# mlpc-ucsd/BDM

Measured on AMD Instinct MI355X. Metric: sampled shapes/sec (4096 pts, 1000 DDPM steps), higher is better.
Workload: dtype f32

## Files before the change

bdm_amd/csrc/common.h:

```cpp
#pragma once
#include <stdlib.h>
#include <hip/hip_runtime.h>
#include <stdint.h>

#define BDM_OK 0
#define BDM_ERR_ARG 1
#define BDM_ERR_LAUNCH 2
#define BDM_ERR_UNSUPPORTED 3

namespace bdm {

void set_error(const char *fmt, ...);

inline int launch_status(const char *what) {
  hipError_t e = hipGetLastError();
  if (e != hipSuccess) {
    set_error("%s: %s (HIP's per-thread last-error state: raised by this launch or left by an earlier unchecked call)",
              what, hipGetErrorString(e));
    return BDM_ERR_LAUNCH;
  }
  return BDM_OK;
}

#define BDM_REQUIRE(cond, ...)      \
// ... 116 lines not shown
__device__ __forceinline__ double wave_sum_bfly(double v) {
  BDM_FULL_WAVE();
  v = row16_sum(v);
  return (readlane_f64(v, 0) + readlane_f64(v, 16)) + (readlane_f64(v, 32) + readlane_f64(v, 48));
}
__device__ __forceinline__ float wave_max(float v) {
  BDM_FULL_WAVE();
  v = fmaxf(v, dpp_f32(v, BDM_DPP_QUAD_XOR1));
  v = fmaxf(v, dpp_f32(v, BDM_DPP_QUAD_XOR2));
  v = fmaxf(v, dpp_f32(v, BDM_DPP_ROW_HALF_MIRROR));
  v = fmaxf(v, dpp_f32(v, BDM_DPP_ROW_MIRROR));
  return fmaxf(fmaxf(readlane_f32(v, 0), readlane_f32(v, 16)), fmaxf(readlane_f32(v, 32), readlane_f32(v, 48)));
}
#endif

struct VoxWs {
  int *start;
  int *tmp;
  int *sorted;
};
static inline VoxWs vox_ws(void *ws, int b, int n, int r3) {
  VoxWs w;
  w.start = (int *)ws;
  w.tmp = w.start + (size_t)b * r3;
  w.sorted = w.tmp + (size_t)b * n;
  return w;
}

#if defined(__HIPCC__)
__device__ __forceinline__ float swishf(float x) {
  return x * __builtin_amdgcn_rcpf(1.0f + __builtin_amdgcn_exp2f(-x * 1.44269504088896340736f));
}
#endif

#if defined(__HIPCC__)
__device__ __forceinline__ void lds_settle(float &a, float &b) { asm volatile("s_waitcnt lgkmcnt(0)" : "+v"(a), "+v"(b)); }
__device__ __forceinline__ void lds_settle8(float (&v)[8]) {
  asm volatile("s_waitcnt lgkmcnt(0)" : "+v"(v[0]), "+v"(v[1]), "+v"(v[2]), "+v"(v[3]), "+v"(v[4]), "+v"(v[5]), "+v"(v[6]), "+v"(v[7]));
}
// ... 4 lines not shown
```

bdm_amd/csrc/pvcnn_ops.hip:

```cpp
#include <stdarg.h>
#include <stdio.h>

#include <stdlib.h>

#include "../../include/bdm_hip.h"
#include "common.h"

#pragma clang fp contract(off)

namespace bdm {
static thread_local char g_err[512] = "";
void set_error(const char *fmt, ...) {
  va_list ap;
  va_start(ap, fmt);
  vsnprintf(g_err, sizeof(g_err), fmt, ap);
  va_end(ap);
}
}

extern "C" const char *bdm_last_error(void) { return bdm::g_err; }
extern "C" int bdm_abi_version(void) { return 4; }

using namespace bdm;

// ... 497 lines not shown
    if (ci < c_a) {
      const float *fr = fa + (size_t)bi * bs_a + (size_t)ci * ld_a;
      out0[(size_t)bi * bs_0 + (size_t)ci * ld_0 + j] =
          __fadd_rn(__fadd_rn(__fmul_rn(fr[i0], w0), __fmul_rn(fr[i1], w1)), __fmul_rn(fr[i2], w2));
    } else if (ci < c_a + c_s) {
      out0[(size_t)bi * bs_0 + (size_t)ci * ld_0 + j] = fs[(size_t)bi * bs_s + (size_t)(ci - c_a) * ld_s + j];
    } else {
      const int ct = ci - c_a - c_s;
      const float *fr = ft + (size_t)bi * bs_t + (size_t)ct * ld_t;
      out1[(size_t)bi * bs_1 + (size_t)ct * ld_1 + j] =
          __fadd_rn(__fadd_rn(__fmul_rn(fr[i0], w0), __fmul_rn(fr[i1], w1)), __fmul_rn(fr[i2], w2));
    }
  }
}

extern "C" int bdm_fp_assemble(int b, int m, int n, const int *indices, const float *weights, int c_a, const float *fa,
                               long long bs_a, int ld_a, int c_s, const float *fs, long long bs_s, int ld_s, int c_t,
                               const float *ft, long long bs_t, int ld_t, float *out0, long long bs_0, int ld_0, float *out1,
                               long long bs_1, int ld_1, void *stream) {
  BDM_REQUIRE(b >= 0 && m >= 1 && n >= 0 && c_a >= 0 && c_s >= 0 && c_t >= 0, "fp_assemble: bad sizes");
  if (b == 0 || n == 0 || c_a + c_s + c_t == 0) return BDM_OK;
  const int c = c_a + c_s + c_t;
  dim3 grid(cdiv(n, 256), c < 64 ? c : 64, b);
  hipLaunchKernelGGL(fp_assemble_kernel, grid, dim3(256), 0, (hipStream_t)stream, n, c_a, fa, bs_a, ld_a, c_s, fs, bs_s, ld_s, c_t,
                     ft, bs_t, ld_t, indices, weights, out0, bs_0, ld_0, out1, bs_1, ld_1);
  return launch_status("fp_assemble");
}

extern "C" int bdm_three_nn_interpolate_forward(int b, int c, int m, int n, const float *points,
                                                const float *centers, const float *features, float *out,
                                                int *indices, float *weights, void *stream) {
  int rc = bdm_three_nn_search(b, m, n, points, centers, indices, weights, stream);
  if (rc) return rc;
  return bdm_three_nn_apply(b, c, m, n, features, (long long)c * m, m, indices, weights, out,
                            (long long)c * n, n, stream);
}

extern "C" size_t bdm_voxelize_workspace_bytes(int b, int n, int r) {
  return sizeof(int) * ((size_t)b * r * r * r + 2 * (size_t)b * n);
}

__global__ void vox_plan_kernel(int n, int r, const int *__restrict__ coords, int *__restrict__ ind,
                                int *__restrict__ cnt, int *__restrict__ start, int *__restrict__ tmp,
                                int *__restrict__ sorted, int n_max, int *__restrict__ occ_index,
                                int *__restrict__ occ_list, int *__restrict__ n_occ, unsigned char *__restrict__ rowocc) {
  extern __shared__ int lcnt[];
  __shared__ int wave_tot[16];
  const int r2 = r * r, r3 = r2 * r;
  const int bi = blockIdx.x, tid = threadIdx.x, T = blockDim.x, lane = tid & 63, wave = tid >> 6;
  const int *vx = coords + (size_t)bi * 3 * n, *vy = vx + n, *vz = vy + n;
  int *id = ind + (size_t)bi * n;
  int *gc = cnt + (size_t)bi * r3;
  int *gs = start + (size_t)bi * r3;
  int *tp = tmp + (size_t)bi * n;
  int *so = sorted + (size_t)bi * n;

  for (int v = tid; v < r3; v += T) lcnt[v] = 0;
  __syncthreads();
  for (int i = tid; i < n; i += T) {
    const int v = vx[i] * r2 + vy[i] * r + vz[i];
// ... 15 lines not shown
  __syncthreads();
  int wave_off = 0;
  for (int w = 0; w < wave; ++w) wave_off += wave_tot[w];
  int run = wave_off + incl - local;
  for (int v = lo; v < hi; ++v) { const int cv = lcnt[v]; gs[v] = run; lcnt[v] = run; run += cv; }
  __syncthreads();
  for (int i = tid; i < n; i += T) tp[atomicAdd(&lcnt[id[i]], 1)] = i;
  __syncthreads();
  for (int i = tid; i < n; i += T) {
    const int v = id[i];
    const int s = gs[v], cv = gc[v];
    int rank = 0;
    for (int q = 0; q < cv; ++q) rank += tp[s + q] < i;
    so[s + rank] = i;
  }
  if (occ_index == nullptr) return;
  __syncthreads();
  int *oi = occ_index + (size_t)bi * r3;
  int *ol = occ_list + (size_t)bi * n_max;
  int occ_local = 0;
  for (int v = lo; v < hi; ++v) occ_local += gc[v] > 0;
  int oincl = occ_local;
#pragma unroll
  for (int o = 1; o < 64; o <<= 1) {
    const int t = __shfl_up(oincl, o, 64);
    if (lane >= o) oincl += t;
  }
  __syncthreads();
  if (lane == 63) wave_tot[wave] = oincl;
  __syncthreads();
  int off = 0, total = 0;
  for (int w = 0; w < (T >> 6); ++w) { if (w < wave) off += wave_tot[w]; total += wave_tot[w]; }
  int orun = off + oincl - occ_local;
  for (int v = lo; v < hi; ++v) {
    if (gc[v] > 0) { oi[v] = orun; ol[orun] = v; ++orun; }
    else oi[v] = -1;
  }
  if (tid == 0) n_occ[bi] = total;
  for (int row = tid; row < r2; row += T) {
    int any = 0;
    for (int z = 0; z < r; ++z) any |= gc[row * r + z];
    rowocc[(size_t)bi * r2 + row] = any ? 1 : 0;
  }
}

template <int CS>
__global__ __launch_bounds__(1024) void vox_plan_slab_kernel(int n, int r, int slabs, const int *__restrict__ coords,
                                                             int *__restrict__ ind, int *__restrict__ cnt,
                                                             int *__restrict__ start, int *__restrict__ sorted, int n_max,
                                                             int *__restrict__ occ_index, int *__restrict__ occ_list,
                                                             int *__restrict__ n_occ, unsigned char *__restrict__ rowocc) {
  extern __shared__ int slab_smem[];
  constexpr int T = 1024, PER = CS / T;
  static_assert(CS % T == 0 && PER >= 1, "slab size must be a multiple of the workgroup size");
  const int r2 = r * r, r3 = r2 * r;
  int *lcnt = slab_smem;
  unsigned *bits = reinterpret_cast<unsigned *>(lcnt + CS);
  int *lbeg = reinterpret_cast<int *>(bits + r3 / 32);
  int *lst = lbeg + CS;
  __shared__ int red[16], red2[16];
  const int bi = blockIdx.x / slabs, sl = blockIdx.x % slabs, tid = threadIdx.x, lane = tid & 63, wave = tid >> 6;
  const int lo_cell = sl * CS;
  const int *vx = coords + (size_t)bi * 3 * n, *vy = vx + n, *vz = vy + n;
  int *id = ind + (size_t)bi * n;
  int *gc = cnt + (size_t)bi * r3, *gs = start + (size_t)bi * r3, *so = sorted + (size_t)bi * n;

  for (int v = tid; v < CS; v += T) lcnt[v] = 0;
  for (int w = tid; w < r3 / 32; w += T) bits[w] = 0u;
  __syncthreads();
  int before = 0;
  for (int i = tid; i < n; i += T) {
    const int v = vx[i] * r2 + vy[i] * r + vz[i];
    if (sl == 0) id[i] = v;
    atomicOr(&bits[v >> 5], 1u << (v & 31));
// ... 6 lines not shown
  __syncthreads();
  int occ_before = 0, occ_total = 0;
  for (int w = tid; w < r3 / 32; w += T) {
    const int pc = __popc(bits[w]);
    occ_total += pc;
    occ_before += (w < lo_cell / 32) ? pc : 0;
  }
#pragma unroll
  for (int o = 32; o > 0; o >>= 1) { occ_before += __shfl_xor(occ_before, o, 64); occ_total += __shfl_xor(occ_total, o, 64); }
  __shared__ int red3[16];
  if (lane == 0) { red2[wave] = occ_before; red3[wave] = occ_total; }
  __syncthreads();
  int point_base = 0, occ_base = 0, occ_all = 0;
  for (int w = 0; w < T / 64; ++w) { point_base += red[w]; occ_base += red2[w]; occ_all += red3[w]; }
  if (sl == 0 && tid == 0 && n_occ != nullptr) n_occ[bi] = occ_all;
  __syncthreads();

  int cv[PER], local = 0, olocal = 0;
#pragma unroll
  for (int j = 0; j < PER; ++j) { cv[j] = lcnt[tid * PER + j]; local += cv[j]; olocal += cv[j] > 0; }
  int incl = local, oincl = olocal;
#pragma unroll
  for (int o = 1; o < 64; o <<= 1) {
    const int t1 = __shfl_up(incl, o, 64), t2 = __shfl_up(oincl, o, 64);
    if (lane >= o) { incl += t1; oincl += t2; }
  }
  if (lane == 63) { red[wave] = incl; red2[wave] = oincl; }
  __syncthreads();
  int woff = 0, owoff = 0;
  for (int w = 0; w < wave; ++w) { woff += red[w]; owoff += red2[w]; }
  int run = woff + incl - local;
  int orun = occ_base + owoff + oincl - olocal;
#pragma unroll
  for (int j = 0; j < PER; ++j) {
    const int v = lo_cell + tid * PER + j;
    gc[v] = cv[j];
    gs[v] = point_base + run;
    lcnt[tid * PER + j] = run;
    lbeg[tid * PER + j] = run;
    if (occ_index != nullptr) {
      if (cv[j] > 0) { occ_index[(size_t)bi * r3 + v] = orun; occ_list[(size_t)bi * n_max + orun] = v; ++orun; }
      else occ_index[(size_t)bi * r3 + v] = -1;
    }
    run += cv[j];
  }
  if (rowocc != nullptr) {
    const int any = local > 0;
    const unsigned long long m = __ballot(any);
    constexpr int TPR_MAX = 64;
    const int tpr = r / PER;
    if (tpr <= TPR_MAX && (lane % tpr) == 0) {
      const unsigned long long rowmask = ((tpr == 64 ? ~0ull : ((1ull << tpr) - 1ull)) << lane);
      const int row = (lo_cell + tid * PER) / r;
      rowocc[(size_t)bi * r2 + row] = (m & rowmask) ? 1 : 0;
    }
  }
  __syncthreads();
  for (int i = tid; i < n; i += T) {
    const int v = vx[i] * r2 + vy[i] * r + vz[i];
    if (v >= lo_cell && v < lo_cell + CS) lst[atomicAdd(&lcnt[v - lo_cell], 1)] = i;
  }
  __syncthreads();
  for (int i = tid; i < n; i += T) {
    const int v = vx[i] * r2 + vy[i] * r + vz[i];
    if (v >= lo_cell && v < lo_cell + CS) {
      const int s0 = lbeg[v - lo_cell], cvv = lcnt[v - lo_cell] - s0;
      int rank = 0;
      for (int q = 0; q < cvv; ++q) rank += lst[s0 + q] < i;
      so[point_base + s0 + rank] = i;
    }
  }
}

__global__ void vox_reduce_kernel(int c, int n, int r3, const float *__restrict__ feat,
                                  const int *__restrict__ cnt, const int *__restrict__ start,
                                  const int *__restrict__ sorted, float *__restrict__ out) {
  const int v = blockIdx.x * blockDim.x + threadIdx.x;
  const int bi = blockIdx.z;
  if (v >= r3) return;
  const int cv = cnt[(size_t)bi * r3 + v];
  const int s = start[(size_t)bi * r3 + v];
  const int *so = sorted + (size_t)bi * n + s;
  const float inv = cv > 0 ? (float)(1.0 / (double)(float)cv) : 0.f;
  for (int ci = blockIdx.y; ci < c; ci += gridDim.y) {
// ... 4 lines not shown
  }
}

static bool vox_plan_slabs() { return bdm_staging_choice() != 0; }

extern "C" int bdm_voxelize_plan(int b, int n, int r, const int *coords, int *ind, int *cnt, void *workspace,
                                 void *stream) {
  BDM_REQUIRE(b >= 0 && n >= 1 && r >= 1 && r <= 32, "voxelize_plan: bad sizes (r<=32 supported)");
  BDM_REQUIRE(workspace != nullptr, "voxelize_plan: workspace is NULL");
  if (b == 0) return BDM_OK;
  const int r3 = r * r * r;
  VoxWs w = vox_ws(workspace, b, n, r3);
  const size_t smem = (size_t)r3 * sizeof(int);
  BDM_ALLOW_LDS(vox_plan_kernel, smem);
  hipLaunchKernelGGL(vox_plan_kernel, dim3(b), dim3(1024), smem, (hipStream_t)stream, n, r, coords, ind, cnt, w.start,
                     w.tmp, w.sorted, 0, (int *)nullptr, (int *)nullptr, (int *)nullptr, (unsigned char *)nullptr);
  return launch_status("vox_plan");
}

extern "C" int bdm_voxelize_plan_full(int b, int n, int r, int n_max, const int *coords, int *ind, int *cnt, void *workspace,
                                      int *occ_index, int *occ_list, int *n_occ, unsigned char *rowocc, void *stream) {
  BDM_REQUIRE(b >= 0 && n >= 1 && r >= 1 && r <= 32 && n_max >= 1, "voxelize_plan_full: bad sizes (r<=32 supported)");
  BDM_REQUIRE(workspace && occ_index && occ_list && n_occ && rowocc, "voxelize_plan_full: NULL buffer");
  if (b == 0) return BDM_OK;
  const int r3 = r * r * r;
  VoxWs w = vox_ws(workspace, b, n, r3);
  if (r == 32 && n <= 24576 && vox_plan_slabs()) {
    const size_t sm = sizeof(int) * (2 * 4096 + (size_t)r3 / 32 + (size_t)n);
    BDM_ALLOW_LDS(vox_plan_slab_kernel<4096>, sm);
    hipLaunchKernelGGL(vox_plan_slab_kernel<4096>, dim3(b * 8), dim3(1024), sm, (hipStream_t)stream, n, r, 8, coords, ind, cnt,
                       w.start, w.sorted, n_max, occ_index, occ_list, n_occ, rowocc);
    return launch_status("vox_plan_full");
  }
  const size_t smem = (size_t)r3 * sizeof(int);
  BDM_ALLOW_LDS(vox_plan_kernel, smem);
  hipLaunchKernelGGL(vox_plan_kernel, dim3(b), dim3(1024), smem, (hipStream_t)stream, n, r, coords, ind, cnt, w.start,
                     w.tmp, w.sorted, n_max, occ_index, occ_list, n_occ, rowocc);
  return launch_status("vox_plan_full");
}

extern "C" int bdm_avg_voxelize_forward(int b, int c, int n, int r, const float *features, const int *coords,
                                        float *out, int *ind, int *cnt, void *workspace, void *stream) {
  BDM_REQUIRE(b >= 0 && c >= 0 && n >= 1 && r >= 1 && r <= 32, "avg_voxelize: bad sizes (r<=32 supported)");
  if (b == 0) return BDM_OK;
  hipStream_t s = (hipStream_t)stream;
  const int r3 = r * r * r;
  int rc = bdm_voxelize_plan(b, n, r, coords, ind, cnt, workspace, stream);
  VoxWs w = vox_ws(workspace, b, n, r3);
  if (rc || c == 0) return rc;
  dim3 grid(cdiv(r3, 256), c < 64 ? c : 64, b);
  hipLaunchKernelGGL(vox_reduce_kernel, grid, dim3(256), 0, s, c, n, r3, features, cnt, w.start, w.sorted, out);
  return launch_status("vox_reduce");
// ... 44 lines not shown
```

bdm_amd/csrc/sparse_conv.hip:

```cpp
#include <stdlib.h>

#include "../../include/bdm_hip.h"
#include "common.h"
#include "s3_split.h"

using namespace bdm;

__global__ void vox_compact_kernel(int r3, int n_max, const int *__restrict__ cnt, int *__restrict__ occ_index,
                                   int *__restrict__ occ_list, int *__restrict__ n_occ) {
  __shared__ int wave_tot[16];
  const int bi = blockIdx.x, tid = threadIdx.x, T = blockDim.x, lane = tid & 63, wave = tid >> 6;
  const int *c = cnt + (size_t)bi * r3;
  int *oi = occ_index + (size_t)bi * r3;
  int *ol = occ_list + (size_t)bi * n_max;
  const int per = (r3 + T - 1) / T;
  const int lo = min(tid * per, r3), hi = min(lo + per, r3);
  int local = 0;
  for (int v = lo; v < hi; ++v) local += c[v] > 0;
  int incl = local;
#pragma unroll
  for (int o = 1; o < 64; o <<= 1) {
    const int t = __shfl_up(incl, o, 64);
    if (lane >= o) incl += t;
  }
// ... 128 lines not shown
#pragma unroll
        for (int j = 0; j < 8; ++j)
          if (j < nch) acc[j] = acc[j] + v[u][j] * inv;
      }
  }
  store_s3(xs + ((size_t)bi * G + g) * 3 * (size_t)n_max * 8, (size_t)k, (size_t)n_max, acc);
}

template <int OUT>
__global__ __launch_bounds__(1024) void sparse_vox_features_lds_kernel(int c, int n, int r3, int n_max, int G, int ksplit,
                                                                       int cells_per,
                                                                       const float *__restrict__ feat, long long bs_f, int ld_f,
                                                                       const int *__restrict__ cnt, const int *__restrict__ start,
                                                                       const int *__restrict__ sorted,
                                                                       const int *__restrict__ occ_list,
                                                                       const int *__restrict__ n_occ, void *__restrict__ outp,
                                                                       unsigned *__restrict__ amax) {
#pragma clang fp contract(off)
  extern __shared__ float frows[];
  constexpr int CPT = 4;
  const int unit = blockIdx.x / ksplit, k0 = (blockIdx.x % ksplit) * cells_per, bi = unit / G, g = unit % G;
  const int tid = threadIdx.x, T = blockDim.x;
  const int nocc = min(n_occ[bi], n_max);
  const int lim = min(OUT == 0 ? min((nocc + 127) & ~127, n_max) : n_max, k0 + cells_per);
  if (k0 >= lim) return;
  const int nch = min(8, c - g * 8);
  const float *fb = feat + (size_t)bi * bs_f + (size_t)g * 8 * ld_f;
  const bool vec = (n & 3) == 0 && (ld_f & 3) == 0 && ((reinterpret_cast<size_t>(fb) & 15) == 0) && (n >> 2) <= T;
  const int n4 = n >> 2;
  float4 rowv[8];
  if (vec) {
#pragma unroll
    for (int j = 0; j < 8; ++j)
      rowv[j] = reinterpret_cast<const float4 *>(fb + (size_t)min(j, nch - 1) * ld_f)[min(tid, n4 - 1)];
  }
  int cs[CPT], cc[CPT];
#pragma unroll
  for (int i = 0; i < CPT; ++i) {
    const int k = k0 + tid + i * T;
    cs[i] = 0; cc[i] = 0;
    if (k < nocc && k < lim) {
      const int v = occ_list[(size_t)bi * n_max + k];
      cc[i] = cnt[(size_t)bi * r3 + v];
      cs[i] = start[(size_t)bi * r3 + v];
    }
  }
  int pre[CPT][4];
#pragma unroll
  for (int i = 0; i < CPT; ++i) {
    const int *so = sorted + (size_t)bi * n + cs[i];
#pragma unroll
    for (int u = 0; u < 4; ++u) pre[i][u] = cc[i] > 0 ? so[min(u, cc[i] - 1)] : 0;
  }
  if (vec) {
    if (tid < n4) {
#pragma unroll
      for (int j = 0; j < 8; ++j)
        reinterpret_cast<float4 *>(frows + j * n)[tid] = j < nch ? rowv[j] : make_float4(0.f, 0.f, 0.f, 0.f);
    }
  } else if ((n & 3) == 0 && (ld_f & 3) == 0 && ((reinterpret_cast<size_t>(fb) & 15) == 0)) {
#pragma unroll
    for (int j = 0; j < 8; ++j) {
      const float4 *src = reinterpret_cast<const float4 *>(fb + (size_t)min(j, nch - 1) * ld_f);
      float4 *dst = reinterpret_cast<float4 *>(frows + j * n);
      for (int p = tid; p < n4; p += T) {
        const float4 v = src[p];
        dst[p] = j < nch ? v : make_float4(0.f, 0.f, 0.f, 0.f);
// ... 6 lines not shown
  __syncthreads();
  float m = 0.f;
#pragma unroll
  for (int i = 0; i < CPT; ++i) {
    const int k = k0 + tid + i * T;
    if (k >= lim) continue;
    const int cv = cc[i];
    const int *so = sorted + (size_t)bi * n + cs[i];
    const float inv = cv > 0 ? (float)(1.0 / (double)(float)cv) : 0.f;
    float acc[8];
#pragma unroll
    for (int j = 0; j < 8; ++j) acc[j] = 0.f;
    for (int q0 = 0; q0 < cv; q0 += 4) {
      int p[4];
#pragma unroll
      for (int u = 0; u < 4; ++u) p[u] = q0 == 0 ? pre[i][u] : so[min(q0 + u, cv - 1)];
#pragma unroll
      for (int u = 0; u < 4; ++u)
        if (q0 + u < cv) {
#pragma unroll
          for (int j = 0; j < 8; ++j) acc[j] = acc[j] + frows[j * n + p[u]] * inv;
        }
    }
    if (OUT == 0) {
      store_s3(reinterpret_cast<unsigned short *>(outp) + ((size_t)bi * G + g) * 3 * (size_t)n_max * 8, (size_t)k, (size_t)n_max, acc);
    } else {
      float4 *o = reinterpret_cast<float4 *>(outp) + (((size_t)bi * G + g) * n_max + k) * 2;
      o[0] = make_float4(acc[0], acc[1], acc[2], acc[3]);
      o[1] = make_float4(acc[4], acc[5], acc[6], acc[7]);
#pragma unroll
      for (int j = 0; j < 8; ++j) m = fmaxf(m, fabsf(acc[j]));
    }
  }
  if (OUT == 1) {
    m = wave_max(m);
    if ((tid & 63) == 0 && m > 0.f) atomicMax(amax + bi, __float_as_uint(m));
  }
}

bool bdm_sparse_features_lds_launch(int out_kind, int b, int c, int n, int r3, int n_max, const float *features, long long bs_f,
                                    int ld_f, const int *cnt, const int *start, const int *sorted, const int *occ_list,
                                    const int *n_occ, void *out, unsigned *amax, hipStream_t stream, int *rc) {
  if (bdm_staging_choice() == 0 || n > 4096 || n_max > 4096) return false;
  const int G = (c + 7) / 8, units = b * G;
  const int ksplit = 1;
  const int cells_per = ((n_max + ksplit - 1) / ksplit + 63) & ~63;
  const int T = cells_per > 1024 ? 1024 : 256;
  const size_t smem = sizeof(float) * 8 * (size_t)n;
  *rc = BDM_OK;
  if (out_kind == 0) {
    static int granted0[16] = {0};
    int dev = 0;
    (void)hipGetDevice(&dev);
    if (smem > 48 * 1024 && (dev < 0 || dev >= 16 || granted0[dev] < (int)smem)) {
      hipError_t e = hipFuncSetAttribute((const void *)sparse_vox_features_lds_kernel<0>, hipFuncAttributeMaxDynamicSharedMemorySize, (int)smem);
      if (e != hipSuccess) return false;
      if (dev >= 0 && dev < 16) granted0[dev] = (int)smem;
    }
    hipLaunchKernelGGL(sparse_vox_features_lds_kernel<0>, dim3(units * ksplit), dim3(T), smem, stream, c, n, r3, n_max, G, ksplit,
                       cells_per, features, bs_f, ld_f, cnt, start, sorted, occ_list, n_occ, out, amax);
  } else {
    static int granted1[16] = {0};
    int dev = 0;
    (void)hipGetDevice(&dev);
    if (smem > 48 * 1024 && (dev < 0 || dev >= 16 || granted1[dev] < (int)smem)) {
      hipError_t e = hipFuncSetAttribute((const void *)sparse_vox_features_lds_kernel<1>, hipFuncAttributeMaxDynamicSharedMemorySize, (int)smem);
      if (e != hipSuccess) return false;
      if (dev >= 0 && dev < 16) granted1[dev] = (int)smem;
    }
    hipLaunchKernelGGL(sparse_vox_features_lds_kernel<1>, dim3(units * ksplit), dim3(T), smem, stream, c, n, r3, n_max, G, ksplit,
                       cells_per, features, bs_f, ld_f, cnt, start, sorted, occ_list, n_occ, out, amax);
  }
  return true;
}

extern "C" int bdm_sparse_voxel_features_s3(int b, int c, int n, int r, int n_max, const float *features, long long bs_f,
                                            int ld_f, const int *cnt, const void *plan_workspace, const int *occ_list,
                                            const int *n_occ, void *xs, void *stream) {
  BDM_REQUIRE(b >= 0 && c >= 1 && n >= 1 && r >= 1 && n_max >= 1, "sparse_voxel_features_s3: bad sizes");
  if (b == 0) return BDM_OK;
  const int r3 = r * r * r;
  VoxWs w = vox_ws(const_cast<void *>(plan_workspace), b, n, r3);
  int rc_lds = BDM_OK;
  if (bdm_sparse_features_lds_launch(0, b, c, n, r3, n_max, features, bs_f, ld_f, cnt, w.start, w.sorted, occ_list, n_occ, xs, nullptr,
                                     (hipStream_t)stream, &rc_lds))
    return launch_status("sparse_voxel_features_s3");
  const int G = (c + 7) / 8, units = b * G, kblocks = cdiv(n_max, 128);
  hipLaunchKernelGGL(sparse_vox_features_s3_kernel, dim3(cdiv(units, 8) * 8 * kblocks), dim3(128), 0, (hipStream_t)stream, c,
                     n, r3, n_max, G, units, kblocks, features, bs_f, ld_f, cnt, w.start, w.sorted, occ_list, n_occ,
                     (unsigned short *)xs);
  return launch_status("sparse_voxel_features_s3");
}

__global__ void sparse_pack_s3_kernel(int cout, int cin, const float *__restrict__ w, unsigned short *__restrict__ ws) {
  const int n27 = 27 * cout, G = (cin + 7) / 8;
  const long long total = (long long)G * n27;
  for (long long e = (long long)blockIdx.x * blockDim.x + threadIdx.x; e < total; e += (long long)gridDim.x * blockDim.x) {
    const int g = (int)(e / n27), col = (int)(e % n27), tap = col / cout, co = col % cout;
    float v[8];
// ... 429 lines not shown
```

bdm_amd/csrc/sparse_conv_h2.hip:

```cpp
#include <stdlib.h>

#include "../../include/bdm_hip.h"
#include "common.h"

using namespace bdm;

#include "sparse_h2_common.h"

bool bdm_sparse_features_lds_launch(int out_kind, int b, int c, int n, int r3, int n_max, const float *features, long long bs_f,
                                    int ld_f, const int *cnt, const int *start, const int *sorted, const int *occ_list,
                                    const int *n_occ, void *out, unsigned *amax, hipStream_t stream, int *rc);

__global__ void sparse_vox_features_f32_kernel(int c, int n, int r3, int n_max, int G, int units, int kblocks,
                                               const float *__restrict__ feat, long long bs_f, int ld_f,
                                               const int *__restrict__ cnt, const int *__restrict__ start,
                                               const int *__restrict__ sorted, const int *__restrict__ occ_list,
                                               const int *__restrict__ n_occ, float4 *__restrict__ xr,
                                               unsigned *__restrict__ amax) {
#pragma clang fp contract(off)
  const int wg = blockIdx.x, span = 8 * kblocks;
  const int unit = (wg / span) * 8 + (wg % span) % 8, kb = (wg % span) / 8;
  if (unit >= units) return;
  const int bi = unit / G, g = unit % G;
  const int k = kb * blockDim.x + threadIdx.x;
  float acc[8];
#pragma unroll
// ... 31 lines not shown
    o[0] = make_float4(acc[0], acc[1], acc[2], acc[3]);
    o[1] = make_float4(acc[4], acc[5], acc[6], acc[7]);
  }
  m = wave_max(m);
  if ((threadIdx.x & 63) == 0 && m > 0.f) atomicMax(amax + bi, __float_as_uint(m));
}

extern "C" int bdm_sparse_voxel_features_f32(int b, int c, int n, int r, int n_max, const float *features, long long bs_f,
                                             int ld_f, const int *cnt, const void *plan_workspace, const int *occ_list,
                                             const int *n_occ, void *xr, float *amax, void *stream) {
  BDM_REQUIRE(b >= 0 && c >= 1 && n >= 1 && r >= 1 && n_max >= 1 && amax != nullptr, "sparse_voxel_features_f32: bad arguments");
  if (b == 0) return BDM_OK;
  const int r3 = r * r * r;
  VoxWs w = vox_ws(const_cast<void *>(plan_workspace), b, n, r3);
  int rc_lds = BDM_OK;
  if (bdm_sparse_features_lds_launch(1, b, c, n, r3, n_max, features, bs_f, ld_f, cnt, w.start, w.sorted, occ_list, n_occ, xr,
                                     (unsigned *)amax, (hipStream_t)stream, &rc_lds))
    return launch_status("sparse_voxel_features_f32");
  const int G = (c + 7) / 8, units = b * G, kblocks = cdiv(n_max, 128);
  hipLaunchKernelGGL(sparse_vox_features_f32_kernel, dim3(cdiv(units, 8) * 8 * kblocks), dim3(128), 0, (hipStream_t)stream, c,
                     n, r3, n_max, G, units, kblocks, features, bs_f, ld_f, cnt, w.start, w.sorted, occ_list, n_occ,
                     (float4 *)xr, (unsigned *)amax);
  return launch_status("sparse_voxel_features_f32");
}

__global__ void sparse_gemm_h2_pack_kernel(int cout, int cin, const float *__restrict__ w, const float *__restrict__ scale,
                                           unsigned short *__restrict__ wq) {
  const int G = (cin + 7) / 8, n27 = 27 * cout;
  const long long total = (long long)G * n27;
  for (long long e = (long long)blockIdx.x * blockDim.x + threadIdx.x; e < total; e += (long long)gridDim.x * blockDim.x) {
    const int col = (int)(e % n27), g = (int)(e / n27), tap = col / cout, co = col % cout;
    unsigned short h[8], l[8];
// ... 167 lines not shown
```

include/bdm_hip.h:

```cpp
#ifndef BDM_HIP_H
#define BDM_HIP_H

#include <stddef.h>
#include <stdint.h>

#ifdef __cplusplus
extern "C" {
#endif

const char *bdm_last_error(void);
int bdm_abi_version(void);


int bdm_furthest_point_sampling(int b, int n, int m, const float *coords, int *indices,
                                float *centers_out, void *stream);

int bdm_gather_features_forward(int b, int c, int n, int m, const float *features,
                                const int *indices, float *out, void *stream);

int bdm_ball_query(int b, int n, int m, float radius, int u, const float *centers,
                   const float *points, int *neighbors, void *stream);

int bdm_grouping_forward(int b, int c, int n, int m, int u, const float *features,
                         const int *indices, float *out, void *stream);

int bdm_fp_assemble(int b, int m, int n, const int *indices, const float *weights, int c_a, const float *fa, long long bs_a,
                    int ld_a, int c_s, const float *fs, long long bs_s, int ld_s, int c_t, const float *ft, long long bs_t,
                    int ld_t, float *out0, long long bs_0, int ld_0, float *out1, long long bs_1, int ld_1, void *stream);
int bdm_three_nn_interpolate_forward(int b, int c, int m, int n, const float *points,
                                     const float *centers, const float *features, float *out,
                                     int *indices, float *weights, void *stream);
int bdm_three_nn_search(int b, int m, int n, const float *points, const float *centers,
                        int *indices, float *weights, void *stream);
int bdm_three_nn_apply(int b, int c, int m, int n, const float *features, long long bs_f, int ld_f,
                       const int *indices, const float *weights, float *out, long long bs_o, int ld_o,
                       void *stream);

size_t bdm_voxelize_workspace_bytes(int b, int n, int r);
int bdm_avg_voxelize_forward(int b, int c, int n, int r, const float *features, const int *coords,
                             float *out, int *ind, int *cnt, void *workspace, void *stream);

int bdm_trilinear_devoxelize_forward(int b, int c, int n, int r, const float *coords,
                                     const float *grid, float *out, void *stream);
// ... 388 lines not shown
```

Measured before the change: 3.117.

## Stage FP interpolation sources in LDS and add per-voxel point records

Adds an LDS-staged feature-propagation kernel. It copies chunks of source feature rows into shared memory, gathers the three-NN weighted sums from there, and vectorises point loads and stores, with a new form-selectable entry point. The voxel plan kernels now also write compact per-occupied-voxel records (count, start and up to six point ids) so the sparse feature kernel can prefetch point indices without an extra indirection. The max reduction now goes through a block-level shared reduction before a guarded atomic. These add workspace, LDS use and plan-kernel writes in exchange for fewer scattered global gathers and fewer atomics.

```diff
diff --git a/bdm_amd/csrc/common.h b/bdm_amd/csrc/common.h
--- a/bdm_amd/csrc/common.h
+++ b/bdm_amd/csrc/common.h
@@ -154,15 +154,27 @@
 }
 #endif
 
+#define VOX_REC 8
+#define VOX_REC_PTS (VOX_REC - 2)
 struct VoxWs {
   int *start;
+  int *rec_flag;
+  int *rec;
   int *tmp;
   int *sorted;
+  int rec_rows;
 };
+static inline size_t vox_ws_rec_offset(int b, int r3) { return ((size_t)b * r3 + (size_t)b + 3) & ~(size_t)3; }
+static inline size_t vox_ws_ints(int b, int n, int r3) {
+  return vox_ws_rec_offset(b, r3) + (size_t)b * (n < r3 ? n : r3) * VOX_REC + 2 * (size_t)b * n;
+}
 static inline VoxWs vox_ws(void *ws, int b, int n, int r3) {
   VoxWs w;
   w.start = (int *)ws;
-  w.tmp = w.start + (size_t)b * r3;
+  w.rec_flag = w.start + (size_t)b * r3;
+  w.rec = w.start + vox_ws_rec_offset(b, r3);
+  w.rec_rows = n < r3 ? n : r3;
+  w.tmp = w.rec + (size_t)b * w.rec_rows * VOX_REC;
   w.sorted = w.tmp + (size_t)b * n;
   return w;
 }
diff --git a/bdm_amd/csrc/pvcnn_ops.hip b/bdm_amd/csrc/pvcnn_ops.hip
--- a/bdm_amd/csrc/pvcnn_ops.hip
+++ b/bdm_amd/csrc/pvcnn_ops.hip
@@ -535,17 +535,161 @@
   }
 }
 
+template <int V>
+__global__ __launch_bounds__(256) void fp_assemble_lds_kernel(int m, int n, int ch, int pts_per, int src_vec, int skip_vec, int c_a,
+                                                              const float *__restrict__ fa, long long bs_a, int ld_a, int c_s,
+                                                              const float *__restrict__ fs, long long bs_s, int ld_s, int c_t,
+                                                              const float *__restrict__ ft, long long bs_t, int ld_t,
+                                                              const int *__restrict__ indices, const float *__restrict__ weights,
+                                                              float *__restrict__ out0, long long bs_0, int ld_0,
+                                                              float *__restrict__ out1, long long bs_1, int ld_1) {
+  extern __shared__ float srow[];
+  const int tid = threadIdx.x, T = blockDim.x, bi = blockIdx.z;
+  const int ka = (c_a + ch - 1) / ch, kt = (c_t + ch - 1) / ch;
+  const int p_lo = blockIdx.x * pts_per, p_hi = min(n, p_lo + pts_per);
+  int y = blockIdx.y;
+  if (y >= ka + kt) {
+    const int c0 = (y - ka - kt) * ch, nc = min(ch, c_s - c0);
+    const float *src = fs + (size_t)bi * bs_s + (size_t)c0 * ld_s;
+    float *dst = out0 + (size_t)bi * bs_0 + (size_t)(c_a + c0) * ld_0;
+    for (int j = p_lo + tid * V; j < p_hi; j += T * V)
+      for (int cc = 0; cc < nc; ++cc) {
+        if (V == 4 && skip_vec) {
+          *reinterpret_cast<float4 *>(dst + (size_t)cc * ld_0 + j) = *reinterpret_cast<const float4 *>(src + (size_t)cc * ld_s + j);
+        } else {
+#pragma unroll
+          for (int u = 0; u < V; ++u) dst[(size_t)cc * ld_0 + j + u] = src[(size_t)cc * ld_s + j + u];
+        }
+      }
+    return;
+  }
+  const bool temb = y >= ka;
+  if (temb) y -= ka;
+  const int c0 = y * ch, nc = min(ch, (temb ? c_t : c_a) - c0);
+  const float *src = temb ? ft + (size_t)bi * bs_t + (size_t)c0 * ld_t : fa + (size_t)bi * bs_a + (size_t)c0 * ld_a;
+  const int ld_src = temb ? ld_t : ld_a;
+  const int ld_dst = temb ? ld_1 : ld_0;
+  float *dst = temb ? out1 + (size_t)bi * bs_1 + (size_t)c0 * ld_1 : out0 + (size_t)bi * bs_0 + (size_t)c0 * ld_0;
+  if (src_vec) {
+    const int m4 = m >> 2;
+    for (int cc = 0; cc < nc; ++cc) {
+      const float4 *s4 = reinterpret_cast<const float4 *>(src + (size_t)cc * ld_src);
+      float4 *d4 = reinterpret_cast<float4 *>(srow + cc * m);
+      for (int p = tid; p < m4; p += T) d4[p] = s4[p];
+    }
+  } else {
+    for (int cc = 0; cc < nc; ++cc)
+      for (int p = tid; p < m; p += T) srow[cc * m + p] = src[(size_t)cc * ld_src + p];
+  }
+  __syncthreads();
+  const int *id = indices + (size_t)bi * 3 * n;
+  const float *w = weights + (size_t)bi * 3 * n;
+  for (int j = p_lo + tid * V; j < p_hi; j += T * V) {
+    int i0[V], i1[V], i2[V];
+    float w0[V], w1[V], w2[V];
+    if constexpr (V == 4) {
+      const int4 a = *reinterpret_cast<const int4 *>(id + j), b4 = *reinterpret_cast<const int4 *>(id + n + j),
+                 c4 = *reinterpret_cast<const int4 *>(id + 2 * (size_t)n + j);
+      const float4 x = *reinterpret_cast<const float4 *>(w + j), y4 = *reinterpret_cast<const float4 *>(w + n + j),
+                   z = *reinterpret_cast<const float4 *>(w + 2 * (size_t)n + j);
+      i0[0] = a.x; i0[1] = a.y; i0[2] = a.z; i0[3] = a.w;
+      i1[0] = b4.x; i1[1] = b4.y; i1[2] = b4.z; i1[3] = b4.w;
+      i2[0] = c4.x; i2[1] = c4.y; i2[2] = c4.z; i2[3] = c4.w;
+      w0[0] = x.x; w0[1] = x.y; w0[2] = x.z; w0[3] = x.w;
+      w1[0] = y4.x; w1[1] = y4.y; w1[2] = y4.z; w1[3] = y4.w;
+      w2[0] = z.x; w2[1] = z.y; w2[2] = z.z; w2[3] = z.w;
+    } else {
+      i0[0] = id[j]; i1[0] = id[n + j]; i2[0] = id[2 * (size_t)n + j];
+      w0[0] = w[j]; w1[0] = w[n + j]; w2[0] = w[2 * (size_t)n + j];
+    }
+#pragma unroll 4
+    for (int cc = 0; cc < nc; ++cc) {
+      const float *fr = srow + cc * m;
+      float o[V];
+#pragma unroll
+      for (int u = 0; u < V; ++u)
+        o[u] = __fadd_rn(__fadd_rn(__fmul_rn(fr[i0[u]], w0[u]), __fmul_rn(fr[i1[u]], w1[u])), __fmul_rn(fr[i2[u]], w2[u]));
+      if constexpr (V == 4) {
+        *reinterpret_cast<float4 *>(dst + (size_t)cc * ld_dst + j) = make_float4(o[0], o[1], o[2], o[3]);
+      } else {
+        dst[(size_t)cc * ld_dst + j] = o[0];
+      }
+    }
+  }
+}
+
+static bool aligned16(const void *p, long long bs, int ld) { return (reinterpret_cast<size_t>(p) & 15) == 0 && (bs & 3) == 0 && (ld & 3) == 0; }
+
+static int fp_assemble_launch(int form, int b, int m, int n, const int *indices, const float *weights, int c_a, const float *fa,
+                              long long bs_a, int ld_a, int c_s, const float *fs, long long bs_s, int ld_s, int c_t, const float *ft,
+                              long long bs_t, int ld_t, float *out0, long long bs_0, int ld_0, float *out1, long long bs_1, int ld_1,
+                              void *stream) {
+  BDM_REQUIRE(b >= 0 && m >= 1 && n >= 0 && c_a >= 0 && c_s >= 0 && c_t >= 0, "fp_assemble: bad sizes");
+  BDM_REQUIRE(form >= 0 && form <= 2, "fp_assemble: form must be 0, 1 or 2");
+  if (b == 0 || n == 0 || c_a + c_s + c_t == 0) return BDM_OK;
+  constexpr int LDS_BUDGET = 32 * 1024, LDS_MAX = 64 * 1024;
+  const bool fits = (size_t)m * 4 <= LDS_MAX && b <= 65535;
+  BDM_REQUIRE(form != 2 || fits, "fp_assemble: the staged form needs m <= 16384 and b <= 65535");
+  if (form == 1 || !fits || (form == 0 && n <= 256)) {
+    const int c = c_a + c_s + c_t;
+    dim3 grid(cdiv(n, 256), c < 64 ? c : 64, b);
+    hipLaunchKernelGGL(fp_assemble_kernel, grid, dim3(256), 0, (hipStream_t)stream, n, c_a, fa, bs_a, ld_a, c_s, fs, bs_s, ld_s, c_t,
+                       ft, bs_t, ld_t, indices, weights, out0, bs_0, ld_0, out1, bs_1, ld_1);
+    return launch_status("fp_assemble");
+  }
+  int ch = LDS_BUDGET / (4 * m);
+  ch = ch < 1 ? 1 : (ch > 8 ? 8 : ch);
+  const int chunks = cdiv(c_a, ch) + cdiv(c_t, ch) + cdiv(c_s, ch);
+  const bool v4 = (n & 3) == 0 && (reinterpret_cast<size_t>(indices) & 15) == 0 && (reinterpret_cast<size_t>(weights) & 15) == 0 &&
+                  (c_a + c_s == 0 || aligned16(out0, bs_0, ld_0)) && (c_t == 0 || aligned16(out1, bs_1, ld_1));
+  const int V = v4 ? 4 : 1;
+  const int src_vec = (m & 3) == 0 && (c_a == 0 || aligned16(fa, bs_a, ld_a)) && (c_t == 0 || aligned16(ft, bs_t, ld_t));
+  const int skip_vec = c_s == 0 || aligned16(fs, bs_s, ld_s);
+  const int T = min(256, max(64, (cdiv(n, V) + 63) & ~63));
+  int cus = 256;
+  {
+    int dev = 0, v = 0;
+    static int cached[16] = {0};
+    (void)hipGetDevice(&dev);
+    if (dev >= 0 && dev < 16) {
+      if (cached[dev] == 0 && hipDeviceGetAttribute(&v, hipDeviceAttributeMultiprocessorCount, dev) == hipSuccess && v > 0) cached[dev] = v;
+      if (cached[dev] > 0) cus = cached[dev];
+    }
+  }
+  const int pass = T * V;
+  long long slices = cdivll(2ll * cus, (long long)b * chunks);
+  slices = slices < 1 ? 1 : slices;
+  if (slices > cdiv(n, pass)) slices = cdiv(n, pass);
+  const int pts_per = cdiv(cdiv(n, (int)slices), pass) * pass;
+  dim3 grid(cdiv(n, pts_per), chunks, b);
+  BDM_REQUIRE(chunks <= 65535, "fp_assemble: too many channels");
+  const size_t smem = sizeof(float) * (size_t)ch * m;
+  if (v4) {
+    BDM_ALLOW_LDS(fp_assemble_lds_kernel<4>, smem);
+    hipLaunchKernelGGL(fp_assemble_lds_kernel<4>, grid, dim3(T), smem, (hipStream_t)stream, m, n, ch, pts_per, src_vec, skip_vec, c_a, fa,
+                       bs_a, ld_a, c_s, fs, bs_s, ld_s, c_t, ft, bs_t, ld_t, indices, weights, out0, bs_0, ld_0, out1, bs_1, ld_1);
+  } else {
+    BDM_ALLOW_LDS(fp_assemble_lds_kernel<1>, smem);
+    hipLaunchKernelGGL(fp_assemble_lds_kernel<1>, grid, dim3(T), smem, (hipStream_t)stream, m, n, ch, pts_per, src_vec, skip_vec, c_a, fa,
+                       bs_a, ld_a, c_s, fs, bs_s, ld_s, c_t, ft, bs_t, ld_t, indices, weights, out0, bs_0, ld_0, out1, bs_1, ld_1);
+  }
+  return launch_status("fp_assemble");
+}
+
 extern "C" int bdm_fp_assemble(int b, int m, int n, const int *indices, const float *weights, int c_a, const float *fa,
                                long long bs_a, int ld_a, int c_s, const float *fs, long long bs_s, int ld_s, int c_t,
                                const float *ft, long long bs_t, int ld_t, float *out0, long long bs_0, int ld_0, float *out1,
                                long long bs_1, int ld_1, void *stream) {
-  BDM_REQUIRE(b >= 0 && m >= 1 && n >= 0 && c_a >= 0 && c_s >= 0 && c_t >= 0, "fp_assemble: bad sizes");
-  if (b == 0 || n == 0 || c_a + c_s + c_t == 0) return BDM_OK;
-  const int c = c_a + c_s + c_t;
-  dim3 grid(cdiv(n, 256), c < 64 ? c : 64, b);
-  hipLaunchKernelGGL(fp_assemble_kernel, grid, dim3(256), 0, (hipStream_t)stream, n, c_a, fa, bs_a, ld_a, c_s, fs, bs_s, ld_s, c_t,
-                     ft, bs_t, ld_t, indices, weights, out0, bs_0, ld_0, out1, bs_1, ld_1);
-  return launch_status("fp_assemble");
+  return fp_assemble_launch(0, b, m, n, indices, weights, c_a, fa, bs_a, ld_a, c_s, fs, bs_s, ld_s, c_t, ft, bs_t, ld_t, out0, bs_0, ld_0,
+                            out1, bs_1, ld_1, stream);
+}
+
+extern "C" int bdm_fp_assemble_form(int form, int b, int m, int n, const int *indices, const float *weights, int c_a, const float *fa,
+                                    long long bs_a, int ld_a, int c_s, const float *fs, long long bs_s, int ld_s, int c_t,
+                                    const float *ft, long long bs_t, int ld_t, float *out0, long long bs_0, int ld_0, float *out1,
+                                    long long bs_1, int ld_1, void *stream) {
+  return fp_assemble_launch(form, b, m, n, indices, weights, c_a, fa, bs_a, ld_a, c_s, fs, bs_s, ld_s, c_t, ft, bs_t, ld_t, out0, bs_0,
+                            ld_0, out1, bs_1, ld_1, stream);
 }
 
 extern "C" int bdm_three_nn_interpolate_forward(int b, int c, int m, int n, const float *points,
@@ -558,13 +702,14 @@
 }
 
 extern "C" size_t bdm_voxelize_workspace_bytes(int b, int n, int r) {
-  return sizeof(int) * ((size_t)b * r * r * r + 2 * (size_t)b * n);
+  return sizeof(int) * vox_ws_ints(b, n, r * r * r);
 }
 
 __global__ void vox_plan_kernel(int n, int r, const int *__restrict__ coords, int *__restrict__ ind,
                                 int *__restrict__ cnt, int *__restrict__ start, int *__restrict__ tmp,
                                 int *__restrict__ sorted, int n_max, int *__restrict__ occ_index,
-                                int *__restrict__ occ_list, int *__restrict__ n_occ, unsigned char *__restrict__ rowocc) {
+                                int *__restrict__ occ_list, int *__restrict__ n_occ, unsigned char *__restrict__ rowocc,
+                                int *__restrict__ rec_flag, int *__restrict__ rec, int rec_rows) {
   extern __shared__ int lcnt[];
   __shared__ int wave_tot[16];
   const int r2 = r * r, r3 = r2 * r;
@@ -610,7 +755,10 @@
     for (int q = 0; q < cv; ++q) rank += tp[s + q] < i;
     so[s + rank] = i;
   }
-  if (occ_index == nullptr) return;
+  if (occ_index == nullptr) {
+    if (tid == 0) rec_flag[bi] = 0;
+    return;
+  }
   __syncthreads();
   int *oi = occ_index + (size_t)bi * r3;
   int *ol = occ_list + (size_t)bi * n_max;
@@ -628,11 +776,21 @@
   int off = 0, total = 0;
   for (int w = 0; w < (T >> 6); ++w) { if (w < wave) off += wave_tot[w]; total += wave_tot[w]; }
   int orun = off + oincl - occ_local;
+  int4 *rc = reinterpret_cast<int4 *>(rec + (size_t)bi * rec_rows * VOX_REC);
   for (int v = lo; v < hi; ++v) {
-    if (gc[v] > 0) { oi[v] = orun; ol[orun] = v; ++orun; }
-    else oi[v] = -1;
-  }
-  if (tid == 0) n_occ[bi] = total;
+    const int cv = gc[v];
+    if (cv > 0) {
+      oi[v] = orun; ol[orun] = v;
+      const int s = gs[v];
+      int pq[VOX_REC_PTS];
+#pragma unroll
+      for (int q = 0; q < VOX_REC_PTS; ++q) pq[q] = q < cv ? so[s + q] : 0;
+      rc[2 * orun] = make_int4(cv, s, pq[0], pq[1]);
+      rc[2 * orun + 1] = make_int4(pq[2], pq[3], pq[4], pq[5]);
+      ++orun;
+    } else oi[v] = -1;
+  }
+  if (tid == 0) { n_occ[bi] = total; rec_flag[bi] = 1; }
   for (int row = tid; row < r2; row += T) {
     int any = 0;
     for (int z = 0; z < r; ++z) any |= gc[row * r + z];
@@ -645,7 +803,8 @@
                                                              int *__restrict__ ind, int *__restrict__ cnt,
                                                              int *__restrict__ start, int *__restrict__ sorted, int n_max,
                                                              int *__restrict__ occ_index, int *__restrict__ occ_list,
-                                                             int *__restrict__ n_occ, unsigned char *__restrict__ rowocc) {
+                                                             int *__restrict__ n_occ, unsigned char *__restrict__ rowocc,
+                                                             int *__restrict__ rec_flag, int *__restrict__ rec, int rec_rows) {
   extern __shared__ int slab_smem[];
   constexpr int T = 1024, PER = CS / T;
   static_assert(CS % T == 0 && PER >= 1, "slab size must be a multiple of the workgroup size");
@@ -653,7 +812,8 @@
   int *lcnt = slab_smem;
   unsigned *bits = reinterpret_cast<unsigned *>(lcnt + CS);
   int *lbeg = reinterpret_cast<int *>(bits + r3 / 32);
-  int *lst = lbeg + CS;
+  int *lrow = lbeg + CS;
+  int *lst = lrow + CS;
   __shared__ int red[16], red2[16];
   const int bi = blockIdx.x / slabs, sl = blockIdx.x % slabs, tid = threadIdx.x, lane = tid & 63, wave = tid >> 6;
   const int lo_cell = sl * CS;
@@ -690,6 +850,8 @@
   int point_base = 0, occ_base = 0, occ_all = 0;
   for (int w = 0; w < T / 64; ++w) { point_base += red[w]; occ_base += red2[w]; occ_all += red3[w]; }
   if (sl == 0 && tid == 0 && n_occ != nullptr) n_occ[bi] = occ_all;
+  if (sl == 0 && tid == 0) rec_flag[bi] = occ_index != nullptr;
+  int *const rc = rec + (size_t)bi * rec_rows * VOX_REC;
   __syncthreads();
 
   int cv[PER], local = 0, olocal = 0;
@@ -715,8 +877,13 @@
     lcnt[tid * PER + j] = run;
     lbeg[tid * PER + j] = run;
     if (occ_index != nullptr) {
-      if (cv[j] > 0) { occ_index[(size_t)bi * r3 + v] = orun; occ_list[(size_t)bi * n_max + orun] = v; ++orun; }
-      else occ_index[(size_t)bi * r3 + v] = -1;
+      if (cv[j] > 0) {
+        occ_index[(size_t)bi * r3 + v] = orun; occ_list[(size_t)bi * n_max + orun] = v;
+        reinterpret_cast<int4 *>(rc)[2 * orun] = make_int4(cv[j], point_base + run, 0, 0);
+        reinterpret_cast<int4 *>(rc)[2 * orun + 1] = make_int4(0, 0, 0, 0);
+        lrow[tid * PER + j] = orun;
+        ++orun;
+      } else occ_index[(size_t)bi * r3 + v] = -1;
     }
     run += cv[j];
   }
@@ -744,6 +911,7 @@
       int rank = 0;
       for (int q = 0; q < cvv; ++q) rank += lst[s0 + q] < i;
       so[point_base + s0 + rank] = i;
+      if (occ_index != nullptr && rank < VOX_REC_PTS) rc[(size_t)lrow[v - lo_cell] * VOX_REC + 2 + rank] = i;
     }
   }
 }
@@ -778,7 +946,8 @@
   const size_t smem = (size_t)r3 * sizeof(int);
   BDM_ALLOW_LDS(vox_plan_kernel, smem);
   hipLaunchKernelGGL(vox_plan_kernel, dim3(b), dim3(1024), smem, (hipStream_t)stream, n, r, coords, ind, cnt, w.start,
-                     w.tmp, w.sorted, 0, (int *)nullptr, (int *)nullptr, (int *)nullptr, (unsigned char *)nullptr);
+                     w.tmp, w.sorted, 0, (int *)nullptr, (int *)nullptr, (int *)nullptr, (unsigned char *)nullptr, w.rec_flag, w.rec,
+                     w.rec_rows);
   return launch_status("vox_plan");
 }
 
@@ -790,16 +959,16 @@
   const int r3 = r * r * r;
   VoxWs w = vox_ws(workspace, b, n, r3);
   if (r == 32 && n <= 24576 && vox_plan_slabs()) {
-    const size_t sm = sizeof(int) * (2 * 4096 + (size_t)r3 / 32 + (size_t)n);
+    const size_t sm = sizeof(int) * (3 * 4096 + (size_t)r3 / 32 + (size_t)n);
     BDM_ALLOW_LDS(vox_plan_slab_kernel<4096>, sm);
     hipLaunchKernelGGL(vox_plan_slab_kernel<4096>, dim3(b * 8), dim3(1024), sm, (hipStream_t)stream, n, r, 8, coords, ind, cnt,
-                       w.start, w.sorted, n_max, occ_index, occ_list, n_occ, rowocc);
+                       w.start, w.sorted, n_max, occ_index, occ_list, n_occ, rowocc, w.rec_flag, w.rec, w.rec_rows);
     return launch_status("vox_plan_full");
   }
   const size_t smem = (size_t)r3 * sizeof(int);
   BDM_ALLOW_LDS(vox_plan_kernel, smem);
   hipLaunchKernelGGL(vox_plan_kernel, dim3(b), dim3(1024), smem, (hipStream_t)stream, n, r, coords, ind, cnt, w.start,
-                     w.tmp, w.sorted, n_max, occ_index, occ_list, n_occ, rowocc);
+                     w.tmp, w.sorted, n_max, occ_index, occ_list, n_occ, rowocc, w.rec_flag, w.rec, w.rec_rows);
   return launch_status("vox_plan_full");
 }
 
diff --git a/bdm_amd/csrc/sparse_conv.hip b/bdm_amd/csrc/sparse_conv.hip
--- a/bdm_amd/csrc/sparse_conv.hip
+++ b/bdm_amd/csrc/sparse_conv.hip
@@ -166,7 +166,9 @@
                                                                        const int *__restrict__ cnt, const int *__restrict__ start,
                                                                        const int *__restrict__ sorted,
                                                                        const int *__restrict__ occ_list,
-                                                                       const int *__restrict__ n_occ, void *__restrict__ outp,
+                                                                       const int *__restrict__ n_occ,
+                                                                       const int *__restrict__ rec_flag, const int *__restrict__ rec,
+                                                                       int rec_rows, void *__restrict__ outp,
                                                                        unsigned *__restrict__ amax) {
 #pragma clang fp contract(off)
   extern __shared__ float frows[];
@@ -174,6 +176,7 @@
   const int unit = blockIdx.x / ksplit, k0 = (blockIdx.x % ksplit) * cells_per, bi = unit / G, g = unit % G;
   const int tid = threadIdx.x, T = blockDim.x;
   const int nocc = min(n_occ[bi], n_max);
+  const bool has_rec = rec_flag[bi] != 0;
   const int lim = min(OUT == 0 ? min((nocc + 127) & ~127, n_max) : n_max, k0 + cells_per);
   if (k0 >= lim) return;
   const int nch = min(8, c - g * 8);
@@ -186,23 +189,35 @@
     for (int j = 0; j < 8; ++j)
       rowv[j] = reinterpret_cast<const float4 *>(fb + (size_t)min(j, nch - 1) * ld_f)[min(tid, n4 - 1)];
   }
-  int cs[CPT], cc[CPT];
-#pragma unroll
-  for (int i = 0; i < CPT; ++i) {
-    const int k = k0 + tid + i * T;
-    cs[i] = 0; cc[i] = 0;
-    if (k < nocc && k < lim) {
-      const int v = occ_list[(size_t)bi * n_max + k];
-      cc[i] = cnt[(size_t)bi * r3 + v];
-      cs[i] = start[(size_t)bi * r3 + v];
-    }
-  }
-  int pre[CPT][4];
-#pragma unroll
-  for (int i = 0; i < CPT; ++i) {
-    const int *so = sorted + (size_t)bi * n + cs[i];
-#pragma unroll
-    for (int u = 0; u < 4; ++u) pre[i][u] = cc[i] > 0 ? so[min(u, cc[i] - 1)] : 0;
+  constexpr int PRE = VOX_REC_PTS;
+  int cs[CPT], cc[CPT], pre[CPT][PRE];
+  if (has_rec) {
+    const int4 *rc = reinterpret_cast<const int4 *>(rec + (size_t)bi * rec_rows * VOX_REC);
+#pragma unroll
+    for (int i = 0; i < CPT; ++i) {
+      const int k = k0 + tid + i * T;
+      int4 a = make_int4(0, 0, 0, 0), b4 = make_int4(0, 0, 0, 0);
+      if (k < nocc && k < lim) { a = rc[2 * k]; b4 = rc[2 * k + 1]; }
+      cc[i] = a.x; cs[i] = a.y;
+      pre[i][0] = a.z; pre[i][1] = a.w; pre[i][2] = b4.x; pre[i][3] = b4.y; pre[i][4] = b4.z; pre[i][5] = b4.w;
+    }
+  } else {
+#pragma unroll
+    for (int i = 0; i < CPT; ++i) {
+      const int k = k0 + tid + i * T;
+      cs[i] = 0; cc[i] = 0;
+      if (k < nocc && k < lim) {
+        const int v = occ_list[(size_t)bi * n_max + k];
+        cc[i] = cnt[(size_t)bi * r3 + v];
+        cs[i] = start[(size_t)bi * r3 + v];
+      }
+    }
+#pragma unroll
+    for (int i = 0; i < CPT; ++i) {
+      const int *so = sorted + (size_t)bi * n + cs[i];
+#pragma unroll
+      for (int u = 0; u < PRE; ++u) pre[i][u] = cc[i] > 0 ? so[min(u, cc[i] - 1)] : 0;
+    }
   }
   if (vec) {
     if (tid < n4) {
@@ -239,7 +254,8 @@
     for (int q0 = 0; q0 < cv; q0 += 4) {
       int p[4];
 #pragma unroll
-      for (int u = 0; u < 4; ++u) p[u] = q0 == 0 ? pre[i][u] : so[min(q0 + u, cv - 1)];
+      for (int u = 0; u < 4; ++u)
+        p[u] = q0 == 0 ? pre[i][u] : (q0 == 4 && u < PRE - 4 ? pre[i][min(4 + u, PRE - 1)] : so[min(q0 + u, cv - 1)]);
 #pragma unroll
       for (int u = 0; u < 4; ++u)
         if (q0 + u < cv) {
@@ -258,45 +274,45 @@
     }
   }
   if (OUT == 1) {
+    __shared__ float wmax[16];
     m = wave_max(m);
-    if ((tid & 63) == 0 && m > 0.f) atomicMax(amax + bi, __float_as_uint(m));
-  }
-}
-
-bool bdm_sparse_features_lds_launch(int out_kind, int b, int c, int n, int r3, int n_max, const float *features, long long bs_f,
-                                    int ld_f, const int *cnt, const int *start, const int *sorted, const int *occ_list,
-                                    const int *n_occ, void *out, unsigned *amax, hipStream_t stream, int *rc) {
-  if (bdm_staging_choice() == 0 || n > 4096 || n_max > 4096) return false;
+    if ((tid & 63) == 0) wmax[tid >> 6] = m;
+    __syncthreads();
+    if (tid == 0) {
+      for (int w = 1; w < (T >> 6); ++w) m = fmaxf(m, wmax[w]);
+      if (m > 0.f && __float_as_uint(m) > __atomic_load_n(amax + bi, __ATOMIC_RELAXED)) atomicMax(amax + bi, __float_as_uint(m));
+    }
+  }
+}
+
+template <int OUT>
+static bool sparse_features_lds_go(int b, int c, int n, int r3, int n_max, const float *features, long long bs_f, int ld_f, const int *cnt,
+                                   const VoxWs &w, const int *occ_list, const int *n_occ, void *out, unsigned *amax, hipStream_t stream) {
   const int G = (c + 7) / 8, units = b * G;
   const int ksplit = 1;
   const int cells_per = ((n_max + ksplit - 1) / ksplit + 63) & ~63;
   const int T = cells_per > 1024 ? 1024 : 256;
   const size_t smem = sizeof(float) * 8 * (size_t)n;
+  static int granted[16] = {0};
+  int dev = 0;
+  (void)hipGetDevice(&dev);
+  if (smem > 48 * 1024 && (dev < 0 || dev >= 16 || granted[dev] < (int)smem)) {
+    hipError_t e = hipFuncSetAttribute((const void *)sparse_vox_features_lds_kernel<OUT>, hipFuncAttributeMaxDynamicSharedMemorySize, (int)smem);
+    if (e != hipSuccess) return false;
+    if (dev >= 0 && dev < 16) granted[dev] = (int)smem;
+  }
+  hipLaunchKernelGGL(sparse_vox_features_lds_kernel<OUT>, dim3(units * ksplit), dim3(T), smem, stream, c, n, r3, n_max, G, ksplit, cells_per,
+                     features, bs_f, ld_f, cnt, w.start, w.sorted, occ_list, n_occ, w.rec_flag, w.rec, w.rec_rows, out, amax);
+  return true;
+}
+
+bool bdm_sparse_features_lds_launch(int out_kind, int b, int c, int n, int r3, int n_max, const float *features, long long bs_f,
+                                    int ld_f, const int *cnt, const bdm::VoxWs &w, const int *occ_list, const int *n_occ, void *out,
+                                    unsigned *amax, hipStream_t stream, int *rc) {
+  if (bdm_staging_choice() == 0 || n > 4096 || n_max > 4096) return false;
   *rc = BDM_OK;
-  if (out_kind == 0) {
-    static int granted0[16] = {0};
-    int dev = 0;
-    (void)hipGetDevice(&dev);
-    if (smem > 48 * 1024 && (dev < 0 || dev >= 16 || granted0[dev] < (int)smem)) {
-      hipError_t e = hipFuncSetAttribute((const void *)sparse_vox_features_lds_kernel<0>, hipFuncAttributeMaxDynamicSharedMemorySize, (int)smem);
-      if (e != hipSuccess) return false;
-      if (dev >= 0 && dev < 16) granted0[dev] = (int)smem;
-    }
-    hipLaunchKernelGGL(sparse_vox_features_lds_kernel<0>, dim3(units * ksplit), dim3(T), smem, stream, c, n, r3, n_max, G, ksplit,
-                       cells_per, features, bs_f, ld_f, cnt, start, sorted, occ_list, n_occ, out, amax);
-  } else {
-    static int granted1[16] = {0};
-    int dev = 0;
-    (void)hipGetDevice(&dev);
-    if (smem > 48 * 1024 && (dev < 0 || dev >= 16 || granted1[dev] < (int)smem)) {
-      hipError_t e = hipFuncSetAttribute((const void *)sparse_vox_features_lds_kernel<1>, hipFuncAttributeMaxDynamicSharedMemorySize, (int)smem);
-      if (e != hipSuccess) return false;
-      if (dev >= 0 && dev < 16) granted1[dev] = (int)smem;
-    }
-    hipLaunchKernelGGL(sparse_vox_features_lds_kernel<1>, dim3(units * ksplit), dim3(T), smem, stream, c, n, r3, n_max, G, ksplit,
-                       cells_per, features, bs_f, ld_f, cnt, start, sorted, occ_list, n_occ, out, amax);
-  }
-  return true;
+  return out_kind == 0 ? sparse_features_lds_go<0>(b, c, n, r3, n_max, features, bs_f, ld_f, cnt, w, occ_list, n_occ, out, amax, stream)
+                       : sparse_features_lds_go<1>(b, c, n, r3, n_max, features, bs_f, ld_f, cnt, w, occ_list, n_occ, out, amax, stream);
 }
 
 extern "C" int bdm_sparse_voxel_features_s3(int b, int c, int n, int r, int n_max, const float *features, long long bs_f,
@@ -307,7 +323,7 @@
   const int r3 = r * r * r;
   VoxWs w = vox_ws(const_cast<void *>(plan_workspace), b, n, r3);
   int rc_lds = BDM_OK;
-  if (bdm_sparse_features_lds_launch(0, b, c, n, r3, n_max, features, bs_f, ld_f, cnt, w.start, w.sorted, occ_list, n_occ, xs, nullptr,
+  if (bdm_sparse_features_lds_launch(0, b, c, n, r3, n_max, features, bs_f, ld_f, cnt, w, occ_list, n_occ, xs, nullptr,
                                      (hipStream_t)stream, &rc_lds))
     return launch_status("sparse_voxel_features_s3");
   const int G = (c + 7) / 8, units = b * G, kblocks = cdiv(n_max, 128);
diff --git a/bdm_amd/csrc/sparse_conv_h2.hip b/bdm_amd/csrc/sparse_conv_h2.hip
--- a/bdm_amd/csrc/sparse_conv_h2.hip
+++ b/bdm_amd/csrc/sparse_conv_h2.hip
@@ -8,8 +8,8 @@
 #include "sparse_h2_common.h"
 
 bool bdm_sparse_features_lds_launch(int out_kind, int b, int c, int n, int r3, int n_max, const float *features, long long bs_f,
-                                    int ld_f, const int *cnt, const int *start, const int *sorted, const int *occ_list,
-                                    const int *n_occ, void *out, unsigned *amax, hipStream_t stream, int *rc);
+                                    int ld_f, const int *cnt, const bdm::VoxWs &w, const int *occ_list, const int *n_occ, void *out,
+                                    unsigned *amax, hipStream_t stream, int *rc);
 
 __global__ void sparse_vox_features_f32_kernel(int c, int n, int r3, int n_max, int G, int units, int kblocks,
                                                const float *__restrict__ feat, long long bs_f, int ld_f,
@@ -71,8 +71,8 @@
   const int r3 = r * r * r;
   VoxWs w = vox_ws(const_cast<void *>(plan_workspace), b, n, r3);
   int rc_lds = BDM_OK;
-  if (bdm_sparse_features_lds_launch(1, b, c, n, r3, n_max, features, bs_f, ld_f, cnt, w.start, w.sorted, occ_list, n_occ, xr,
-                                     (unsigned *)amax, (hipStream_t)stream, &rc_lds))
+  if (bdm_sparse_features_lds_launch(1, b, c, n, r3, n_max, features, bs_f, ld_f, cnt, w, occ_list, n_occ, xr, (unsigned *)amax,
+                                     (hipStream_t)stream, &rc_lds))
     return launch_status("sparse_voxel_features_f32");
   const int G = (c + 7) / 8, units = b * G, kblocks = cdiv(n_max, 128);
   hipLaunchKernelGGL(sparse_vox_features_f32_kernel, dim3(cdiv(units, 8) * 8 * kblocks), dim3(128), 0, (hipStream_t)stream, c,
diff --git a/include/bdm_hip.h b/include/bdm_hip.h
--- a/include/bdm_hip.h
+++ b/include/bdm_hip.h
@@ -27,6 +27,10 @@
 int bdm_fp_assemble(int b, int m, int n, const int *indices, const float *weights, int c_a, const float *fa, long long bs_a,
                     int ld_a, int c_s, const float *fs, long long bs_s, int ld_s, int c_t, const float *ft, long long bs_t,
                     int ld_t, float *out0, long long bs_0, int ld_0, float *out1, long long bs_1, int ld_1, void *stream);
+int bdm_fp_assemble_form(int form, int b, int m, int n, const int *indices, const float *weights, int c_a, const float *fa,
+                         long long bs_a, int ld_a, int c_s, const float *fs, long long bs_s, int ld_s, int c_t, const float *ft,
+                         long long bs_t, int ld_t, float *out0, long long bs_0, int ld_0, float *out1, long long bs_1, int ld_1,
+                         void *stream);
 int bdm_three_nn_interpolate_forward(int b, int c, int m, int n, const float *points,
                                      const float *centers, const float *features, float *out,
                                      int *indices, float *weights, void *stream);
```

Result: faster. 3.152 (median of 6 runs) (+1.2%).
